# Medical-Image-Analysis-Laboratory/fetal_t2mapping

Measured on AMD Instinct MI355X. Metric: Mvoxel/s T2 fit, 256³×8TE 3-param LM, 1/2/4/8 GPU; % HBM roofline, higher is better.
Workload: dtype f64

## Files before the change

fetal_t2mapping_amd/csrc/t2fit_kernels.hip:

```cpp
#include <hip/hip_runtime.h>

#include <algorithm>
#include <atomic>
#include <cstdlib>
#include <string>

#include "t2fit_config.h"
#include "t2fit_diag.h"
#include "t2fit_dispatch.h"
#include "t2fit_error.h"
#include "t2fit_launch.h"
#include "t2fit_support.h"

using namespace t2fit;

namespace {

constexpr int kLdsStride = kBlock + 1;
#ifndef T2_SAMPLE_LOAD
#define T2_SAMPLE_LOAD(p) (*(p))
#endif
#ifndef T2_WAVE_HINT
#define T2_WAVE_HINT 2
#endif
constexpr int kWaveHint = T2_WAVE_HINT;

struct Tuning {
  bool use_persistent = true;
  int persistent_blocks = 2048;
  int refill_min = 0;
  bool nte_special = true;
  int take = 0;
  int64_t small_volume = 1 << 20;
  int wave_wg = 1;
  int waves_per_cu = 0;
};
std::atomic<bool> g_reserve_set{false};
std::atomic<int> g_reserve_cus{0};

const Tuning& tuning() {
  static const Tuning tuned = [] {
    Tuning t;
    if (const char* e = std::getenv("T2FIT_ONE_SHOT")) t.use_persistent = std::atoi(e) == 0;
    if (const char* e = std::getenv("T2FIT_PERSISTENT_BLOCKS")) t.persistent_blocks = std::max(1, std::atoi(e));
    if (const char* e = std::getenv("T2FIT_REFILL_MIN")) t.refill_min = std::min(64, std::max(1, std::atoi(e)));
    if (const char* e = std::getenv("T2FIT_RESERVE_CUS"); e && !g_reserve_set.load()) g_reserve_cus.store(std::max(0, std::atoi(e)));
    if (const char* e = std::getenv("T2FIT_NTE_SPECIAL")) t.nte_special = std::atoi(e) != 0;
    if (const char* e = std::getenv("T2FIT_TAKE")) t.take = std::max(0, std::min(64, std::atoi(e)));
    if (const char* e = std::getenv("T2FIT_SMALL_VOLUME")) t.small_volume = std::max<int64_t>(0, std::atoll(e));
    if (const char* e = std::getenv("T2FIT_WAVE_WG")) t.wave_wg = std::max(0, std::atoi(e));
    if (const char* e = std::getenv("T2FIT_WAVES_PER_CU")) t.waves_per_cu = std::max(0, std::atoi(e));
    return t;
  }();
  return tuned;
}

thread_local bool g_timing = false;
constexpr int kEvRing = 16;
thread_local hipEvent_t g_ev0[kEvRing] = {}, g_ev1[kEvRing] = {}, g_ev2[kEvRing] = {};
thread_local long g_ev_count = 0;
thread_local int g_ev_slot = 0;

double event_ms(int launches_ago, const hipEvent_t* from, const hipEvent_t* to) {
  if (launches_ago < 0 || launches_ago >= kEvRing || launches_ago >= g_ev_count) return -1.0;
  const int slot = (int)((g_ev_count - 1 - launches_ago) % kEvRing);
  if (hipEventSynchronize(to[slot]) != hipSuccess) return -1.0;
  float ms = 0.0f;
  if (hipEventElapsedTime(&ms, from[slot], to[slot]) != hipSuccess) return -1.0;
  return (double)ms;
}

struct DevMaps {
  float *t2, *k, *sigma, *res, *r2, *fun, *se;
  int32_t* nit;
  uint8_t* status;
  double* xd;
  double* fund;
  double* trace = nullptr;
  int32_t* trace_len = nullptr;
  int trace_cap = 0;
};

__device__ __forceinline__ void stage_echoes(float* lds, const float* __restrict__ echoes, int layout,
                                             int n_te, int64_t n_vox, int64_t base, bool load_own) {
  const int lane = threadIdx.x;
  if (layout == T2FIT_LAYOUT_TE_MAJOR) {
    if (load_own) {
      const float* src = echoes + base + lane;
      for (int i = 0; i < n_te; ++i) lds[i * kLdsStride + lane] = src[(int64_t)i * n_vox];
    }
  } else {
    const int64_t rows = n_vox - base < kBlock ? n_vox - base : kBlock;
    const int total = (int)rows * n_te;
    const float* src = echoes + base * n_te;
    for (int j = lane; j < total; j += kBlock) {
      const int v = j / n_te;
      const int i = j - v * n_te;
      lds[i * kLdsStride + v] = src[j];
    }
    __syncthreads();
  }
}

template <bool kExtras = true, bool kEpilogueFollows = false>
__device__ __forceinline__ void store_masked(const DevMaps& m, int64_t v) {
  m.t2[v] = 0.0f; m.k[v] = 0.0f; m.sigma[v] = 0.0f;
  if constexpr (!kEpilogueFollows) m.res[v] = 0.0f;
  if constexpr (!kExtras) return;
  if constexpr (!kEpilogueFollows) {
    if (m.r2) m.r2[v] = 0.0f;
    if (m.se) m.se[v] = 0.0f;
  }
  if (m.fun) m.fun[v] = 0.0f;
  if (m.nit) m.nit[v] = 0;
  if (m.status) m.status[v] = T2FIT_ST_MASKED;
  if (m.xd) { m.xd[3 * v] = 0.0; m.xd[3 * v + 1] = 0.0; m.xd[3 * v + 2] = 0.0; }
  if (m.fund) m.fund[v] = 0.0;
}

__device__ __forceinline__ void store_result(const DevMaps& m, int64_t v, const LaneOutputs& o, const LaneResult& r) {
  m.t2[v] = o.t2; m.k[v] = o.k; m.sigma[v] = o.sigma; m.res[v] = o.res;
  if (m.r2) m.r2[v] = o.r2;
  if (m.se) m.se[v] = o.se;
  if (m.fun) m.fun[v] = o.fun;
  if (m.nit) m.nit[v] = o.nit;
  if (m.status) m.status[v] = o.status;
  if (m.xd) { m.xd[3 * v] = r.x[0]; m.xd[3 * v + 1] = r.x[1]; m.xd[3 * v + 2] = r.x[2]; }
  if (m.fund) m.fund[v] = r.fun;
}

template <bool kExtras = true>
__device__ __forceinline__ void store_fit(const DevMaps& m, int64_t v, const LaneResult& r) {
  m.k[v] = (float)r.x[0]; m.t2[v] = (float)r.x[1]; m.sigma[v] = (float)r.x[2];
  if constexpr (!kExtras) return;
  if (m.fun) m.fun[v] = (float)r.fun;
  if (m.nit) m.nit[v] = r.nit;
  if (m.status) m.status[v] = r.status;
  if (m.xd) { m.xd[3 * v] = r.x[0]; m.xd[3 * v + 1] = r.x[1]; m.xd[3 * v + 2] = r.x[2]; }
  if (m.fund) m.fund[v] = r.fun;
}

template <int SOLVER, int PREC, int MODEL>
__global__ __launch_bounds__(kBlock) void fit_volume_kernel(const LaneParams P, const float* __restrict__ echoes,
                                                            int layout, const uint8_t* __restrict__ mask,
                                                            int64_t n_vox, DevMaps m) {
  extern __shared__ float lds[];
  const int lane = threadIdx.x;
  const int64_t base = (int64_t)blockIdx.x * kBlock;
  const int64_t v = base + lane;
  const bool in_range = v < n_vox;
  const bool active = in_range && (mask == nullptr || mask[v] != 0);
  stage_echoes(lds, echoes, layout, P.n_te, n_vox, base, active);
  if (!in_range) return;
  if (!active) {
    store_masked(m, v);
    return;
  }
  bool finite;
  float y0_raw;
  const ObjCtx c = prepare_samples(P, lds + lane, kLdsStride, finite, y0_raw);
  LaneResult r;
  fit_lane_t<SOLVER, PREC, MODEL>(P, c, finite, y0_raw, r);
  LaneOutputs o;
  lane_epilogue(c, r, o, m.r2 != nullptr, m.se != nullptr);
  store_result(m, v, o, r);
}

constexpr int kLoglinVec = 4;
constexpr int kLoglinTile = kBlock * kLoglinVec;

template <bool kExtras>
__global__ __launch_bounds__(kBlock) void loglin_volume_kernel(const LaneParams P, const float* __restrict__ echoes,
                                                               const uint8_t* __restrict__ mask, int64_t n_vox,
                                                               DevMaps m) {
  extern __shared__ float lds[];
  const int lane = threadIdx.x;
  const int64_t v0 = (int64_t)blockIdx.x * kLoglinTile + (int64_t)lane * kLoglinVec;
  if (v0 >= n_vox) return;
  const int n_te = P.n_te;
  bool act[kLoglinVec] = {true, true, true, true};
  if (mask) {
    const uchar4 mk = *reinterpret_cast<const uchar4*>(mask + v0);
    act[0] = mk.x != 0; act[1] = mk.y != 0; act[2] = mk.z != 0; act[3] = mk.w != 0;
  }
  const bool any = act[0] || act[1] || act[2] || act[3];
  bool fin[kLoglinVec] = {true, true, true, true};
  float ymax[kLoglinVec] = {0.0f, 0.0f, 0.0f, 0.0f}, y0[kLoglinVec] = {0.0f, 0.0f, 0.0f, 0.0f};
  if (any) {
    const float* src = echoes + v0;
    for (int i0 = 0; i0 < n_te; i0 += 8) {
      float4 tmp[8];
#pragma unroll
      for (int j = 0; j < 8; ++j)
        if (i0 + j < n_te) tmp[j] = *reinterpret_cast<const float4*>(src + (int64_t)(i0 + j) * n_vox);
#pragma unroll
      for (int j = 0; j < 8; ++j)
        if (i0 + j < n_te) {
          float* dst = lds + (i0 + j) * kLoglinTile + lane;
          const float sv[kLoglinVec] = {tmp[j].x, tmp[j].y, tmp[j].z, tmp[j].w};
#pragma unroll
          for (int q = 0; q < kLoglinVec; ++q) {
            dst[q * kBlock] = sv[q];
            fin[q] = fin[q] && t2_finite(sv[q]);
            if (i0 + j == 0) { y0[q] = sv[q]; ymax[q] = sv[q]; }
            ymax[q] = sv[q] > ymax[q] ? sv[q] : ymax[q];
          }
        }
    }
  }
  float o_t2[kLoglinVec], o_k[kLoglinVec], o_res[kLoglinVec];
  const bool want_fun = kExtras && (m.fun != nullptr || m.fund != nullptr);
#pragma unroll
  for (int q = 0; q < kLoglinVec; ++q) {
    o_t2[q] = 0.0f; o_k[q] = 0.0f; o_res[q] = 0.0f;
    const int64_t v = v0 + q;
    if (!act[q]) {
      if constexpr (kExtras) {
        if (m.r2) m.r2[v] = 0.0f;
        if (m.se) m.se[v] = 0.0f;
        if (m.fun) m.fun[v] = 0.0f;
        if (m.nit) m.nit[v] = 0;
        if (m.status) m.status[v] = T2FIT_ST_MASKED;
        if (m.xd) { m.xd[3 * v] = 0.0; m.xd[3 * v + 1] = 0.0; m.xd[3 * v + 2] = 0.0; }
        if (m.fund) m.fund[v] = 0.0;
      }
      continue;
    }
    float* col = lds + q * kBlock + lane;
    bool finite = fin[q];
    if (P.norm) {
      for (int i = 0; i < n_te; ++i) {
        const float sv = col[i * kLoglinTile] / ymax[q];
        col[i * kLoglinTile] = sv;
        finite = finite && t2_finite(sv);
      }
    }
    ObjCtx c;
    c.P = &P;
    c.y = EchoView{col, kLoglinTile};
    double lb[3], ub[3];
    const bool feasible = lane_bounds(P, y0[q], lb, ub);
    LaneResult r;
    r.nit = 0; r.nfev = 0; r.fun = NAN;
    if (!feasible) {
      r.x[0] = NAN; r.x[1] = NAN; r.x[2] = 0.0;
      r.status = T2FIT_ST_INFEASIBLE;
    } else if (!finite) {
      r.x[0] = t2_clip(P.x0[0], lb[0], ub[0]); r.x[1] = t2_clip(P.x0[1], lb[1], ub[1]); r.x[2] = 0.0;
      r.status = T2FIT_ST_NONFINITE;
    } else {
      loglin_solve(c, lb, ub, want_fun, r);
    }
    LaneOutputs o;
    lane_epilogue(c, r, o, kExtras && m.r2 != nullptr, kExtras && m.se != nullptr);
    o_t2[q] = o.t2; o_k[q] = o.k; o_res[q] = o.res;
    if constexpr (kExtras) {
      if (m.r2) m.r2[v] = o.r2;
      if (m.se) m.se[v] = o.se;
      if (m.fun) m.fun[v] = o.fun;
      if (m.nit) m.nit[v] = o.nit;
      if (m.status) m.status[v] = o.status;
      if (m.xd) { m.xd[3 * v] = r.x[0]; m.xd[3 * v + 1] = r.x[1]; m.xd[3 * v + 2] = r.x[2]; }
      if (m.fund) m.fund[v] = r.fun;
    }
  }
  *reinterpret_cast<float4*>(m.t2 + v0) = make_float4(o_t2[0], o_t2[1], o_t2[2], o_t2[3]);
  *reinterpret_cast<float4*>(m.k + v0) = make_float4(o_k[0], o_k[1], o_k[2], o_k[3]);
  *reinterpret_cast<float4*>(m.sigma + v0) = make_float4(0.0f, 0.0f, 0.0f, 0.0f);
  *reinterpret_cast<float4*>(m.res + v0) = make_float4(o_res[0], o_res[1], o_res[2], o_res[3]);
}

constexpr int kChunkLarge = 256;
constexpr int kChunkSmall = 64;
constexpr int kQueueCap = 64 + kChunkLarge;

template <int MODEL, int NTE = 0, int HOME = PAIRS_LDS> struct LbfgsbLane {
  using Solver = Lbfgsb<MODEL, NTE, HOME>;
  using WaveWg = LbfgsbLane<MODEL, NTE, MODEL == T2FIT_MODEL_GAUSSIAN ? PAIRS_LDS
                                         : MODEL == T2FIT_MODEL_RICIAN ? PAIRS_GLOBAL : PAIRS_REG>;
  static constexpr bool kGlobalPart = Solver::kPairGlobal;
  static constexpr int NP = Solver::N;
  static constexpr int kNte = NTE;
  static constexpr int kHistDoubles = Solver::M * Solver::PAIR_L;
  static constexpr int kWavesPerSimd = 1;
  static constexpr bool kWaveWgOk = true;
#ifndef T2_WAVE_HINT_2PAR
#define T2_WAVE_HINT_2PAR 3
#endif
  static constexpr int kWaveWgHint = MODEL == T2FIT_MODEL_GAUSSIAN ? T2_WAVE_HINT_2PAR : kWaveHint;
  static constexpr int kRefillMin = MODEL == T2FIT_MODEL_RICIAN ? 4 : 8;
  static constexpr bool kSplit = true;
  __device__ static void init(Solver& s, const ObjCtx&, const double* x0, const double* lb, const double* ub,
                              double* hist, int hstride, double* ghist) { s.init(x0, lb, ub, hist, hstride, ghist, 64); }
  __device__ static void result(const Solver& s, const ObjCtx&, LaneResult& r) { s.result(r); }
  template <int J> __device__ static void take_sample(Solver& s, float y) {
    if constexpr (NTE > 0 && J < NTE) s.ys[J] = y;
  }
};
template <typename T, int NPAR, int NTE = 0> struct LmLaneAdaptor {
  using Solver = LmLane<T, NPAR, NTE>;
  using WaveWg = LmLaneAdaptor<T, NPAR, NTE>;
  static constexpr bool kGlobalPart = false;
  static constexpr int NP = NPAR;
  static constexpr int kNte = NTE;
  static constexpr int kHistDoubles = 0;
  static constexpr bool kWaveWgOk = false;
  static constexpr int kWaveWgHint = 1;
  static constexpr int kWavesPerSimd = sizeof(T) == 4 ? 4 : 1;
  static constexpr int kRefillMin = 24;
  static constexpr bool kSplit = false;
  __device__ static void init(Solver& s, const ObjCtx& c, const double* x0, const double* lb, const double* ub,
                              double*, int, double*) { s.init(c, x0, lb, ub); }
  __device__ static void result(const Solver& s, const ObjCtx& c, LaneResult& r) { s.result(c, r); }
  template <int J> __device__ static void take_sample(Solver&, float) {}
};

template <class A, int kChunk, bool kTrace, bool kExtras, int kWg = kBlock, bool kRegs = false>
__device__ __forceinline__ void persistent_fit(const LaneParams& P, const float* __restrict__ echoes, int layout,
                                               const uint8_t* __restrict__ mask, int64_t n_vox, const DevMaps& m,
                                               unsigned long long* next_chunk, int refill_min, int take, double* ghist_all) {
  extern __shared__ float lds[];
  constexpr int NP = A::NP;
  constexpr bool kWaveWg = kRegs;
  static_assert(kRegs ? (kChunk == 64 && A::kNte > 0 && A::kNte <= 8) : kWg == kBlock,
                "workgroup of 256 lanes, or waves taking 64-voxel chunks with the samples in registers");
  constexpr int kStride = kWaveWg ? 64 : kLdsStride;
  const int lane = threadIdx.x & 63, wave = threadIdx.x >> 6;
  float* col = lds + threadIdx.x;
  double* hist = reinterpret_cast<double*>(lds + (kWaveWg ? 0 : ((P.n_te * kStride + 1) & ~1))) + threadIdx.x;
  uint32_t* queue = reinterpret_cast<uint32_t*>(hist - threadIdx.x + A::kHistDoubles * kWg) + wave * kQueueCap;
  double* ghist = nullptr;
  if constexpr (A::kGlobalPart)
    ghist = ghist_all + ((size_t)blockIdx.x * (kWg / 64) + wave) * (A::Solver::M * 64) + lane;
  uint32_t qv = 0;
  const unsigned long long lt_mask = lane == 0 ? 0ull : (~0ull >> (64 - lane));
  const EchoView y{col, kStride};
  int q_head = 0, q_count = 0;
  bool chunks_left = true;
  bool busy = false, done = false;
  int64_t v = 0;
  typename A::Solver s;
  ObjCtx c;
  c.P = &P;
  c.y = y;
  double box_x0[3], box_lb[3], box_ub[3];
#pragma unroll
  for (int j = 0; j < 3; ++j) { box_x0[j] = P.x0[j]; box_lb[j] = P.lb[j]; box_ub[j] = P.ub[j]; }
  T2_STAMPS_BEGIN(queue - wave * kQueueCap + (kBlock / 64) * kQueueCap, wave, lane, c)
  T2_RECORD_PLACEMENT(next_chunk, blockIdx.x * (kWg / 64) + wave, lane)
  bool parked = false;
  int pend = 0;
  const int kTake = take;
  int64_t base_a = 0;
  int sub_a = 0;
  uint32_t idx_b = 0;
  uint8_t mask_a = 0;
  auto load_mask = [&](int64_t base) -> uint8_t {
    const int64_t vv = base + lane;
    return vv < n_vox ? (mask ? mask[vv] : (uint8_t)1) : (uint8_t)0;
  };
  if constexpr (kWaveWg) {
    uint32_t c0 = 0;
    if (lane == 0) c0 = (uint32_t)atomicAdd(next_chunk, 1ull);
    base_a = (int64_t)__shfl(c0, 0, 64) * (64 * kTake);
    mask_a = load_mask(base_a);
    if (lane == 0) idx_b = (uint32_t)atomicAdd(next_chunk, 1ull);
  }
  for (;;) {
    unsigned long long need = __ballot(!busy);
    if (__popcll(need) >= refill_min || need == ~0ull) {
      do {
      T2_BLK_T0(t_rf)
      if (done) {
        LaneResult r;
        A::result(s, c, r);
        store_fit<kExtras>(m, v, r);
        done = false;
      }
      bool fresh = false;
      if constexpr (kWaveWg) {
        unsigned long long want = need;
        for (;;) {
          if (q_count == 0) {
            if (!chunks_left) break;
            const int64_t base = base_a;
            if (base >= n_vox) { chunks_left = false; break; }
            const int64_t vv = base + lane;
            const bool act = mask_a != 0;
            if (++sub_a < kTake) {
              base_a += 64;
              mask_a = load_mask(base_a);
            } else {
              sub_a = 0;
              base_a = (int64_t)__shfl(idx_b, 0, 64) * (64 * kTake);
              mask_a = load_mask(base_a);
              if (lane == 0) idx_b = (uint32_t)atomicAdd(next_chunk, 1ull);
            }
            const unsigned long long b = __ballot(act);
            q_count = __popcll(b);
            q_head = 0;
            const int dst = act ? __popcll(b & lt_mask) : q_count + __popcll(~b & lt_mask);
            qv = (uint32_t)__builtin_amdgcn_ds_permute(dst << 2, (int)(uint32_t)vv);
            if (vv < n_vox && !act) store_masked<kExtras, true>(m, vv);
            if (q_count == 0) continue;
          }
          const int rank = __popcll(want & lt_mask);
          const uint32_t got = (uint32_t)__builtin_amdgcn_ds_bpermute(((q_head + rank) & 63) << 2, (int)qv);
          if (!busy && rank < q_count) {
            v = (int64_t)got;
            busy = true;
            fresh = true;
          }
          const int n_want = __popcll(want);
          const int taken = n_want < q_count ? n_want : q_count;
          q_head += taken;
          q_count -= taken;
          want = __ballot(!busy);
          if (want == 0ull) break;
        }
      } else {
      const int n_need = __popcll(need);
      while (q_count < n_need && chunks_left) {
        unsigned long long cidx = 0;
        if (lane == 0) cidx = atomicAdd(next_chunk, 1ull);
        cidx = __shfl(cidx, 0, 64);
        const int64_t base = (int64_t)cidx * kChunk;
        if (base >= n_vox) { chunks_left = false; break; }
        if (q_head != 0) {
          uint32_t tmp = 0;
          if (lane < q_count) tmp = queue[q_head + lane];
          if (lane < q_count) queue[lane] = tmp;
          q_head = 0;
        }
        bool act[kChunk / 64];
#pragma unroll
        for (int q = 0; q < kChunk / 64; ++q) {
          const int64_t vv = base + q * 64 + lane;
          act[q] = vv < n_vox && (mask == nullptr || mask[vv] != 0);
        }
#pragma unroll
        for (int q = 0; q < kChunk / 64; ++q) {
          const unsigned long long b = __ballot(act[q]);
          if (act[q]) queue[q_count + __popcll(b & lt_mask)] = (uint32_t)(base + q * 64 + lane);
          q_count += __popcll(b);
        }
#pragma unroll
        for (int q = 0; q < kChunk / 64; ++q) {
          const int64_t vv = base + q * 64 + lane;
          if (vv < n_vox && !act[q]) store_masked<kExtras, true>(m, vv);
        }
      }
      if (!busy) {
        const int rank = __popcll(need & lt_mask);
        if (rank < q_count) {
          v = (int64_t)queue[q_head + rank];
          busy = true;
          fresh = true;
        }
      }
      const int taken = n_need < q_count ? n_need : q_count;
      q_head += taken;
      q_count -= taken;
      }
      if (fresh) {
        bool finite = true;
        float ymax = 0.0f, y0 = 0.0f;
        const int n_te = A::kNte > 0 ? A::kNte : P.n_te;
        float first8[8] = {};
        for (int i0 = 0; i0 < n_te; i0 += 8) {
          float tmp[8];
#pragma unroll
          for (int j = 0; j < 8; ++j)
            if (i0 + j < n_te)
              tmp[j] = T2_SAMPLE_LOAD(layout == T2FIT_LAYOUT_TE_MAJOR ? &echoes[(int64_t)(i0 + j) * n_vox + v]
                                                                      : &echoes[v * n_te + (i0 + j)]);
#pragma unroll
          for (int j = 0; j < 8; ++j)
            if (i0 + j < n_te) {
              const float sv = tmp[j];
              if constexpr (!kWaveWg) col[(i0 + j) * kStride] = sv;
              if (i0 == 0) first8[j] = sv;
              finite = finite && t2_finite(sv);
              if (i0 + j == 0) { y0 = sv; ymax = sv; }
              ymax = sv > ymax ? sv : ymax;
            }
        }
        if (P.norm) {
          if constexpr (A::kNte > 0) {
#pragma unroll
            for (int j = 0; j < 8; ++j)
              if (j < n_te) {
                const float sv = first8[j] / ymax;
                first8[j] = sv;
                if constexpr (!kWaveWg) col[j * kStride] = sv;
                finite = finite && t2_finite(sv);
              }
          } else {
            for (int i = 0; i < n_te; ++i) {
              const float sv = col[i * kStride] / ymax;
              col[i * kStride] = sv;
              finite = finite && t2_finite(sv);
            }
          }
        }
        if constexpr (A::kNte > 0)
          static_for<0, 8>([&](auto JC) { A::template take_sample<decltype(JC)::value>(s, first8[decltype(JC)::value]); });
        double lb[3], ub[3];
#pragma unroll
        for (int j = 0; j < 3; ++j) { lb[j] = box_lb[j]; ub[j] = box_ub[j]; }
        if (P.no_prior) {
          lb[0] = (double)y0; ub[0] = P.np_k_ub;
          lb[1] = P.np_t2_lb; ub[1] = P.np_t2_ub;
        }
        bool feasible = true;
#pragma unroll
        for (int j = 0; j < NP; ++j) feasible = feasible && !(lb[j] > ub[j]);
        if (!feasible || !finite) {
          LaneResult r;
          r.nit = 0; r.nfev = 0; r.fun = NAN;
          for (int j = 0; j < 3; ++j)
            r.x[j] = !feasible ? (j < NP ? NAN : 0.0) : (j < NP ? t2_clip(box_x0[j], lb[j], ub[j]) : 0.0);
          r.status = !feasible ? T2FIT_ST_INFEASIBLE : T2FIT_ST_NONFINITE;
          store_fit<kExtras>(m, v, r);
          busy = false;
        } else {
          if constexpr (kTrace) {
            c.trace = m.trace + (size_t)v * 4 * m.trace_cap;
            c.trace_cap = m.trace_cap;
            c.trace_n = m.trace_len + v;
            *c.trace_n = 0;
          }
          A::init(s, c, box_x0, lb, ub, hist, kWg, ghist);
          if constexpr (A::kSplit) { T2_STAMPS_ATTACH(s) }
        }
      }
      T2_BLK_END(c, 8, t_rf)
      need = __ballot(!busy);
      } while (need == ~0ull && (chunks_left || q_count != 0));
    }
    if (__ballot(busy) == 0ull) break;
    if constexpr (A::kSplit) {
      if (busy) {
        if (!parked) {
          T2_BLK_T0(t_ev)
          s.eval(c);
          T2_BLK_END(c, 7, t_ev)
          pend = s.digest(c);
        }
        if (pend == A::Solver::GO_BEGIN || pend == A::Solver::GO_FAIL) {
          T2_BLK_T0(t_bg)
          pend = s.begin_pass(c, pend);
          T2_BLK_END(c, 9, t_bg)
        }
        parked = pend == A::Solver::GO_BEGIN || pend == A::Solver::GO_FAIL;
        if (pend == A::Solver::GO_DONE) { busy = false; done = true; }
      }
    } else {
      if (busy) s.eval(c);
      if (busy && s.advance(c)) {
        busy = false;
        done = true;
      }
    }
  }
  if (done) {
    LaneResult r;
    A::result(s, c, r);
    store_fit<kExtras>(m, v, r);
  }
  T2_STAMPS_END(next_chunk, lane)
}

template <class A, int kChunk, bool kTrace = false, int kWavesPerSimd = 1, bool kExtras = true, int kWg = kBlock,
          bool kRegs = false>
__global__ __launch_bounds__(kWg, kWavesPerSimd) void fit_persistent_kernel(const LaneParams P,
                                                                    const float* __restrict__ echoes, int layout,
                                                                    const uint8_t* __restrict__ mask, int64_t n_vox,
                                                                    DevMaps m, unsigned long long* next_chunk, int refill_min,
                                                                    int take, double* ghist) {
  persistent_fit<A, kChunk, kTrace, kExtras, kWg, kRegs>(P, echoes, layout, mask, n_vox, m, next_chunk, refill_min, take, ghist);
}

__global__ __launch_bounds__(kBlock) void residuals_kernel(const LaneParams P, const float* __restrict__ echoes,
                                                           int layout, const uint8_t* __restrict__ mask,
                                                           int64_t n_vox, const float* __restrict__ t2,
                                                           const float* __restrict__ k,
                                                           const float* __restrict__ sigma, float* res, float* r2,
                                                           float* se) {
  extern __shared__ float lds[];
  const int lane = threadIdx.x;
  const int64_t base = (int64_t)blockIdx.x * kBlock;
  const int64_t v = base + lane;
  const bool in_range = v < n_vox;
  const bool active = in_range && (mask == nullptr || mask[v] != 0);
  stage_echoes(lds, echoes, layout, P.n_te, n_vox, base, active);
  if (!in_range) return;
  float out = 0.0f, out2 = 0.0f, out3 = 0.0f;
  if (active) {
    bool finite;
    float y0_raw;
    const ObjCtx c = prepare_samples(P, lds + lane, kLdsStride, finite, y0_raw);
    const float kv = k[v], tv = t2[v], sv = sigma ? sigma[v] : 0.0f;
    out = residual_mean(c, kv, tv, sv);
    if (r2) out2 = r_squared(c, (double)kv, (double)tv, (double)sv);
    if (se) out3 = t2_std_error(c, (double)kv, (double)tv, (double)sv);
  }
  res[v] = out;
  if (r2) r2[v] = out2;
  if (se) se[v] = out3;
}

using FitKernel = void (*)(const LaneParams, const float*, int, const uint8_t*, int64_t, DevMaps);

FitKernel pick_kernel(const t2fit_config& c) {
  if (c.solver == T2FIT_SOLVER_LM) {
// ... 259 lines not shown
```

fetal_t2mapping_amd/csrc/t2fit_lane.h:

```cpp
#pragma once

#include <math.h>
#include <stdint.h>

#include <type_traits>

#include "../../include/t2fit.h"
#include "t2fit_diag.h"

#if defined(__HIPCC__)
#define T2_HD __host__ __device__ __forceinline__
#define T2_DEVICE_COMPILE 1
#define T2_UNROLL _Pragma("unroll")
#else
#define T2_HD inline
#define T2_UNROLL
#endif

namespace t2fit {

struct LaneParams {
  int32_t model, solver, precision, n_te;
  int32_t no_prior, norm, maxls, maxiter, maxfun, numpy_legacy;
  double te[T2FIT_MAX_TE];
// ... 82 lines not shown
  double r = fma(-0x1.62e42fefa39efp-1, n, x);
  r = fma(-0x1.abc9e3b39803fp-56, n, r);
  double p = fma(0x1.ade156a5dcb37p-26, r, 0x1.28af3fca7ab0cp-22);
  p = fma(r, p, 0x1.71dee623fde64p-19);
  p = fma(r, p, 0x1.a01997c89e6b0p-16);
  p = fma(r, p, 0x1.a01a014761f6ep-13);
  p = fma(r, p, 0x1.6c16c1852b7b0p-10);
  p = fma(r, p, 0x1.1111111122322p-7);
  p = fma(r, p, 0x1.55555555502a1p-5);
  p = fma(r, p, 0x1.5555555555511p-3);
  p = fma(r, p, 0x1.000000000000bp-1);
  p = fma(r, p, 1.0);
  p = fma(r, p, 1.0);
  return __builtin_ldexp(p, (int)n);
}
T2_HD double t2_sqrt_core(double x) {
  const double y = fmin(__builtin_amdgcn_rsq(x), 1e300);
  double g = x * y, h = y * 0.5;
  const double r = fma(-h, g, 0.5);
  g = fma(g, r, g);
  double d = fma(-g, g, x);
  h = fma(h, r, h);
  g = fma(d, h, g);
  d = fma(-g, g, x);
  g = fma(d, h, g);
  return g;
}
#else
T2_HD double t2_exp_core(double x) { return exp(x); }
T2_HD double t2_sqrt_core(double x) { return sqrt(x); }
#endif

T2_HD double t2_sqrt_from_seed_seq(double x, double y, double& h_out) {
  double g = x * y, h = y * 0.5;
  const double r = fma(-h, g, 0.5);
  g = fma(g, r, g);
  double d = fma(-g, g, x);
  h = fma(h, r, h);
  g = fma(d, h, g);
  d = fma(-g, g, x);
  g = fma(d, h, g);
  h_out = h;
  return g;
}
T2_HD double t2_rsqrt_half_near_seq(double a, double h) {
  const double g = a * (h + h);
  return fma(h, fma(-h, g, 0.5), h);
}
T2_HD double t2_sqrt_near_seq(double a, double h) {
  double g = a * (h + h);
  const double r = fma(-h, g, 0.5);
  g = fma(g, r, g);
  const double hi = fma(h, r, h);
  const double d = fma(-g, g, a);
  return fma(d, hi, g);
}
T2_HD double t2_sqrt_from_h_seq(double a, double h) {
  const double g0 = a * (h + h);
  return fma(fma(-g0, g0, a), h, g0);
}
#if defined(__HIP_DEVICE_COMPILE__)
T2_HD double t2_sqrt_core_h(double x, double& h_out) { return t2_sqrt_from_seed_seq(x, __builtin_amdgcn_rsq(x), h_out); }
T2_HD double t2_sqrt_near(double a, double h) { return t2_sqrt_near_seq(a, h); }
T2_HD double t2_rsqrt_half_near(double a, double h) { return t2_rsqrt_half_near_seq(a, h); }
T2_HD double t2_sqrt_from_h(double a, double h) { return t2_sqrt_from_h_seq(a, h); }
#else
T2_HD double t2_sqrt_core_h(double x, double& h_out) { h_out = 0.5 / sqrt(x); return sqrt(x); }
T2_HD double t2_sqrt_near(double a, double) { return sqrt(a); }
T2_HD double t2_rsqrt_half_near(double a, double) { return 0.5 / sqrt(a); }
T2_HD double t2_sqrt_from_h(double a, double) { return sqrt(a); }
#endif

template <typename T> T2_HD T t2_min(T a, T b) { return a < b ? a : b; }
template <typename T> T2_HD T t2_max(T a, T b) { return a > b ? a : b; }
template <typename T> T2_HD T t2_clip(T x, T lo, T hi) {
  T r = x;
  if (lo > r) r = lo;
  if (hi < r) r = hi;
  return r;
}
template <typename T> T2_HD T t2_abs(T a) { return a < T(0) ? -a : a; }
T2_HD bool t2_finite(double x) { return (x - x) == 0.0; }
T2_HD bool t2_finite(float x) { return (x - x) == 0.0f; }

template <typename T> struct TeOf;
template <> struct TeOf<double> {
  T2_HD static double at(const LaneParams& P, int i) { return P.te[i]; }
};
template <> struct TeOf<float> {
  T2_HD static float at(const LaneParams& P, int i) { return P.te_f[i]; }
};

template <int J, int JN, class F> T2_HD void static_for(F&& f) {
  if constexpr (J < JN) {
    f(std::integral_constant<int, J>{});
    static_for<J + 1, JN>(f);
  }
}

#if defined(__HIPCC__)
#define T2_TABLE __device__ __constant__
#else
#define T2_TABLE static const
#endif
T2_TABLE double t2_i0e_A[30] = {
    -4.41534164647933937950E-18, 3.33079451882223809783E-17,  -2.43127984654795469359E-16,
    1.71539128555513303061E-15,  -1.16853328779934516808E-14, 7.67618549860493561688E-14,
    -4.85644678311192946090E-13, 2.95505266312963983461E-12,  -1.72682629144155570723E-11,
    9.67580903537323691224E-11,  -5.18979560163526290666E-10, 2.65982372468238665035E-9,
    -1.30002500998624804212E-8,  6.04699502254191894932E-8,   -2.67079385394061173391E-7,
    1.11738753912010371815E-6,   -4.41673835845875056359E-6,  1.64484480707288970893E-5,
    -5.75419501008210370398E-5,  1.88502885095841655729E-4,   -5.76375574538582365885E-4,
    1.63947561694133579842E-3,   -4.32430999505057594430E-3,  1.05464603945949983183E-2,
    -2.37374148058994688156E-2,  4.93052842396707084878E-2,   -9.49010970480476444210E-2,
    1.71620901522208775349E-1,   -3.04682672343198398683E-1,  6.76795274409476084995E-1};
T2_TABLE double t2_i0e_B[25] = {
    -7.23318048787475395456E-18, -4.83050448594418207126E-18, 4.46562142029675999901E-17,
    3.46122286769746109310E-17,  -2.82762398051658348494E-16, -3.42548561967721913462E-16,
    1.77256013305652638360E-15,  3.81168066935262242075E-15,  -9.55484669882830764870E-15,
    -4.15056934728722208663E-14, 1.54008621752140982691E-14,  3.85277838274214270114E-13,
    7.18012445138366623367E-13,  -1.79417853150680611778E-12, -1.32158118404477131188E-11,
    -3.14991652796324136454E-11, 1.18891471078464383424E-11,  4.94060238822496958910E-10,
    3.39623202570838634515E-9,   2.26666899049817806459E-8,   2.04891858946906374183E-7,
    2.89137052083475648297E-6,   6.88975834691682398426E-5,   3.36911647825569408990E-3,
    8.04490411014108831608E-1};

#if defined(T2_I0E_FMA)
#define T2_CLENSHAW(z, b1, b2, c) (fma(z, b1, -(b2)) + (c))
#else
#define T2_CLENSHAW(z, b1, b2, c) ((z) * (b1) - (b2) + (c))
#endif
#if defined(__HIP_DEVICE_COMPILE__)
#define T2_NOUNROLL _Pragma("nounroll")
#define T2_WAVE_ANY(p) (__ballot(p) != 0ull)
#else
#define T2_NOUNROLL
#define T2_WAVE_ANY(p) (p)
#endif

T2_HD double t2_chbevl(double x, const double* c, int n) {
  double b0 = c[0], b1 = 0.0, b2 = 0.0;
  for (int i = 1; i < n; ++i) {
    b2 = b1;
    b1 = b0;
    b0 = x * b1 - b2 + c[i];
  }
  return 0.5 * (b0 - b2);
}

T2_HD double t2_i0e(double x) {
  if (x < 0) x = -x;
  if (x <= 8.0) return t2_chbevl(x * 0.5 - 2.0, t2_i0e_A, 30);
  return t2_fdiv(t2_chbevl(t2_fdiv(32.0, x) - 2.0, t2_i0e_B, 25), t2_sqrt_core(x));
}

T2_HD void t2_chbevl4(const double* z, const double* tab, int chunks, double* out) {
  double b0[4], b1[4], b2[4];
  T2_UNROLL
  for (int j = 0; j < 4; ++j) { b0[j] = 0.0; b1[j] = 0.0; b2[j] = 0.0; }
  double cn[5];
  T2_UNROLL
  for (int q = 0; q < 5; ++q) cn[q] = tab[q];
  T2_NOUNROLL
  for (int it = 0; it < chunks; ++it) {
    double cc[5];
    T2_UNROLL
// ... 295 lines not shown
```

fetal_t2mapping_amd/csrc/t2fit_lbfgsb.h:

```cpp
#pragma once

#include <type_traits>

#include "t2fit_lane.h"

namespace t2fit {

template <int MODEL> struct ObjTerm;
T2_HD double rician_log_term(float log_y, double log_s2, bool legacy) {
  return legacy ? (double)(log_y - (float)log_s2) : (double)log_y - log_s2;
}
template <> struct ObjTerm<T2FIT_MODEL_GAUSSIAN> {
  double k, t2;
  T2_HD void set(const ObjCtx&, const double* x) { k = x[0]; t2 = x[1]; }
  T2_HD double at(const ObjCtx& c, int i) const {
    const double r = (double)c.sample(i) - k * t2_exp_core(t2_fdiv(-c.P->te[i], t2));
    return r * r;
  }
  T2_HD double finish(const ObjCtx& c, double s) const { return s / c.P->n_te; }
};
template <> struct ObjTerm<T2FIT_MODEL_GAUSSIAN_RICIAN> {
  double k2, t2, s2;
  T2_HD void set(const ObjCtx&, const double* x) { k2 = x[0] * x[0]; t2 = x[1]; s2 = x[2] * x[2]; }
  T2_HD double at(const ObjCtx& c, int i) const {
// ... 692 lines not shown
    T2_UNROLL
    for (int i = 0; i < N; ++i) { fr[i] = iwhere[i] <= 0; nfree += fr[i]; du[i] = 0.0; }
    T2_UNROLL
    for (int i = 0; i < N; ++i) {
      double bz = 0.0;
      T2_UNROLL
      for (int j = 0; j < N; ++j) bz = fma(B[i][j], z[j] - x[j], bz);
      r[i] = fr[i] ? -(g[i] + bz) : 0.0;
    }
    double A[3][3] = {{1, 0, 0}, {0, 1, 0}, {0, 0, 1}};
    T2_UNROLL
    for (int i = 0; i < N; ++i)
      T2_UNROLL
      for (int j = 0; j < N; ++j)
        if (fr[i] && fr[j]) A[i][j] = B[i][j];
    double rr[3] = {r[0], r[1], N == 3 ? r[N - 1] : 0.0};
    if (N == 2) rr[2] = 0.0;
    const double d0 = A[0][0], r0 = t2_fast_rcp(d0);
    const double l10 = A[1][0] * r0, l20 = A[2][0] * r0;
    const double d1 = fma(-l10, A[1][0], A[1][1]), r1 = t2_fast_rcp(d1);
    const double a21 = fma(-l20, A[1][0], A[2][1]);
    const double l21 = a21 * r1;
    const double d2 = fma(-l21, a21, fma(-l20, A[2][0], A[2][2])), r2 = t2_fast_rcp(d2);
    const bool pos_def = (d0 > 0.0) & (d1 > 0.0) & (d2 > 0.0);
    const double y0 = rr[0], y1 = fma(-l10, y0, rr[1]), y2 = fma(-l21, y1, fma(-l20, y0, rr[2]));
    const double u2 = y2 * r2, u1 = fma(-l21, u2, y1 * r1);
    const double u0 = fma(-l20, u2, fma(-l10, u1, y0 * r0));
    du[0] = u0; du[1] = u1;
    if (N == 3) du[N - 1] = u2;
    double xp[N];
    bool projected = false;
    T2_UNROLL
    for (int i = 0; i < N; ++i) {
      xp[i] = z[i];
      const double xk = lb_min(ub[i], lb_max(lb[i], z[i] + du[i]));
      z[i] = fr[i] ? xk : z[i];
      projected = projected | (fr[i] & ((xk == lb[i]) | (xk == ub[i])));
    }
    double ddp = 0.0;
    T2_UNROLL
    for (int i = 0; i < N; ++i) ddp = fma(z[i] - x[i], g[i], ddp);
    if (projected && ddp > 0.0) {
      T2_UNROLL
      for (int i = 0; i < N; ++i) z[i] = xp[i];
      double alpha = 1.0, temp1 = 1.0;
      bool hit[N];
      T2_UNROLL
      for (int i = 0; i < N; ++i) hit[i] = false;
      T2_UNROLL
      for (int i = 0; i < N; ++i) {
        if (fr[i]) {
          const double dk = du[i];
          if (dk < 0.0) {
            const double temp2 = lb[i] - z[i];
            if (temp2 >= 0.0) temp1 = 0.0;
            else if (dk * alpha < temp2) temp1 = t2_fdiv(temp2, dk);
          } else if (dk > 0.0) {
            const double temp2 = ub[i] - z[i];
            if (temp2 <= 0.0) temp1 = 0.0;
            else if (dk * alpha > temp2) temp1 = t2_fdiv(temp2, dk);
          }
          if (temp1 < alpha) {
            alpha = temp1;
            T2_UNROLL
            for (int j = 0; j < N; ++j) hit[j] = j == i;
          }
        }
      }
      if (alpha < 1.0) {
        T2_UNROLL
        for (int i = 0; i < N; ++i)
          if (hit[i]) {
            if (du[i] > 0.0) { z[i] = ub[i]; du[i] = 0.0; }
            else if (du[i] < 0.0) { z[i] = lb[i]; du[i] = 0.0; }
          }
      }
      T2_UNROLL
      for (int i = 0; i < N; ++i)
        if (fr[i]) z[i] = fma(alpha, du[i], z[i]);
    }
    return pos_def;
  }

  T2_HD void init(const double* x0_, const double* lb_, const double* ub_, double* hist_, int hstride_,
                  double* ghist_ = nullptr, int gstride_ = 0) {
    hist = hist_;
    hstride = hstride_;
    ghist = ghist_;
    gstride = gstride_;
    head = 0;
    T2_UNROLL
    for (int i = 0; i < N; ++i) {
      lb[i] = lb_[i];
      ub[i] = ub_[i];
      x[i] = t2_clip(x0_[i], lb[i], ub[i]);
      iwhere[i] = (ub[i] - lb[i] <= 0.0) ? 3 : 0;
    }
    col = 0; nit = 0; nfev = 0; ifun = 0;
    theta = 1.0;
    status = T2FIT_ST_NOT_CONV;
    first = true;
    wn_stale = false;
    T2_UNROLL
    for (int i = 0; i < N; ++i) { z[i] = 0.0; d[i] = 0.0; t[i] = 0.0; r[i] = 0.0; g[i] = 0.0; }
    f = 0.0; fold = 0.0; gd = 0.0; gdold = 0.0; stp = 1.0; stpmx = 1.0; sbgnrm = 0.0;
    ls.task = LS_START; ls.stage = 1; ls.brackt = false;
    ls.ginit = ls.gtest = ls.gx = ls.gy = ls.finit = ls.fx = ls.fy = 0.0;
    ls.stx = ls.sty = ls.stmin = ls.stmax = ls.width = ls.width1 = 0.0;
  }

  enum { GO_BEGIN, GO_TRIAL, GO_FAIL, GO_DONE };

  T2_HD int digest(const ObjCtx& c) {
    const LaneParams& P = *c.P;
    const double epsmch = 2.220446049250313e-16;
    T2_BLK_T0(t_dig)
    const bool was_first = first;
    first = false;
    double gdn = 0.0;
    T2_UNROLL
    for (int i = 0; i < N; ++i) gdn += g[i] * d[i];
    LsState lsn = ls;
    const int task = dcsrch_tests(f, gdn, stp, 0.9, 0.1, 0.0, stpmx, lsn);
    const bool cont = !was_first & (task == LS_FG);
    const bool newit = !was_first & (task != LS_FG);
    double stpn = stp;
    dcsrch_update(f, gdn, stpn, 0.1, 0.0, stpmx, lsn);
    const double sb = projgr(x, g);
    const double tol = P.lbfgsb_tol;
    const int nit1 = nit + 1;
    const bool out_of_budget = (nit1 >= P.maxiter) | (nfev > P.maxfun);
    const bool converged = (sb <= P.gtol) | (!was_first & ((fold - f) <= tol * t2_max3(lb_abs(fold), lb_abs(f), 1.0)));
    double rn[N], dn[N], rr = 0.0;
    T2_UNROLL
    for (int i = 0; i < N; ++i) { rn[i] = g[i] - r[i]; rr += rn[i] * rn[i]; }
    const double dr = (gdn - gdold) * stp, ddum = -gdold * stp;
    T2_UNROLL
    for (int i = 0; i < N; ++i) dn[i] = d[i] * stp;
    const double theta_n = t2_fdiv(rr, dr);
    const double rsy = t2_fast_rsqrt(dr);
    const bool iterate_on = newit & !out_of_budget & !converged;
    const bool store_pair = iterate_on & !(dr <= epsmch * ddum);
    if (!was_first) gd = gdn;
    if (cont) { ls = lsn; stp = stpn; ++ifun; }
    if (!cont && !was_first) ls.task = lsn.task;
    if (was_first || newit) sbgnrm = sb;
    if (newit) {
      nit = nit1;
      if (c.trace && *c.trace_n < c.trace_cap) {
        double* tr = c.trace + 4 * (*c.trace_n)++;
        tr[0] = x[0]; tr[1] = x[1]; tr[2] = N == 3 ? x[N - 1] : 0.0; tr[3] = f;
      }
    }
    if (iterate_on) {
      T2_UNROLL
      for (int i = 0; i < N; ++i) { r[i] = rn[i]; d[i] = dn[i]; }
    }
    if (store_pair) {
      if (col == M) {
        head = (head + 1) % M;
        col = M - 1;
      }
      const int q = slot_of(col);
      store_s(q, dn);
      T2_UNROLL
      for (int i = 0; i < N; ++i) hy(q, i) = rn[i] * rsy;
      ++col;
      theta = theta_n;
    }
    if ((was_first || newit) && converged && !(newit && out_of_budget)) status = T2FIT_ST_CONVERGED;
    const int next_ls = ifun - 1 >= P.maxls ? GO_FAIL : GO_TRIAL;
    const int next_it = (converged | (!was_first & out_of_budget)) ? GO_DONE : GO_BEGIN;
    const int next = cont ? next_ls : next_it;
    T2_BLK_END(c, 0, t_dig)
    set_trial(next == GO_TRIAL);
    return next;
  }

  T2_HD void set_trial(bool on = true) {
    T2_UNROLL
    for (int i = 0; i < N; ++i) {
      const double xt = stp * d[i] + t[i];
      x[i] = on ? (stp == 1.0 ? z[i] : xt) : x[i];
    }
  }
// ... 98 lines not shown
```

Baseline: 1629.

## Streamline wave-workgroup refill: 32-bit offsets, early sample loads, skip scratch zeroing

In the wave-per-workgroup L-BFGS-B path, the refill step now issues the echo sample loads before storing the previous voxel's result, so memory latency overlaps the stores. It uses 32-bit byte offsets for map stores and TE-major sample loads when the volume has fewer than 2^30 voxels, and replaces per-sample finiteness checks with a bitwise max-magnitude test. Solver scratch state is zeroed once per lane rather than on every voxel init, and the refill threshold for non-Rician models drops from 8 to 6. The change depends on the solver never reading stale scratch values between voxels, and adds code paths for the two offset and layout cases.

```diff
diff --git a/fetal_t2mapping_amd/csrc/t2fit_kernels.hip b/fetal_t2mapping_amd/csrc/t2fit_kernels.hip
--- a/fetal_t2mapping_amd/csrc/t2fit_kernels.hip
+++ b/fetal_t2mapping_amd/csrc/t2fit_kernels.hip
@@ -102,9 +102,14 @@
   }
 }
 
-template <bool kExtras = true, bool kEpilogueFollows = false>
+template <bool kOff32> __device__ __forceinline__ float& map_at(float* map, int64_t v) {
+  if constexpr (kOff32) return *reinterpret_cast<float*>(reinterpret_cast<char*>(map) + ((uint32_t)v << 2));
+  else return map[v];
+}
+
+template <bool kExtras = true, bool kEpilogueFollows = false, bool kOff32 = false>
 __device__ __forceinline__ void store_masked(const DevMaps& m, int64_t v) {
-  m.t2[v] = 0.0f; m.k[v] = 0.0f; m.sigma[v] = 0.0f;
+  map_at<kOff32>(m.t2, v) = 0.0f; map_at<kOff32>(m.k, v) = 0.0f; map_at<kOff32>(m.sigma, v) = 0.0f;
   if constexpr (!kEpilogueFollows) m.res[v] = 0.0f;
   if constexpr (!kExtras) return;
   if constexpr (!kEpilogueFollows) {
@@ -129,9 +134,9 @@
   if (m.fund) m.fund[v] = r.fun;
 }
 
-template <bool kExtras = true>
+template <bool kExtras = true, bool kOff32 = false>
 __device__ __forceinline__ void store_fit(const DevMaps& m, int64_t v, const LaneResult& r) {
-  m.k[v] = (float)r.x[0]; m.t2[v] = (float)r.x[1]; m.sigma[v] = (float)r.x[2];
+  map_at<kOff32>(m.k, v) = (float)r.x[0]; map_at<kOff32>(m.t2, v) = (float)r.x[1]; map_at<kOff32>(m.sigma, v) = (float)r.x[2];
   if constexpr (!kExtras) return;
   if (m.fun) m.fun[v] = (float)r.fun;
   if (m.nit) m.nit[v] = r.nit;
@@ -288,10 +293,14 @@
 #define T2_WAVE_HINT_2PAR 3
 #endif
   static constexpr int kWaveWgHint = MODEL == T2FIT_MODEL_GAUSSIAN ? T2_WAVE_HINT_2PAR : kWaveHint;
-  static constexpr int kRefillMin = MODEL == T2FIT_MODEL_RICIAN ? 4 : 8;
+  static constexpr int kRefillMin = MODEL == T2FIT_MODEL_RICIAN ? 4 : 6;
   static constexpr bool kSplit = true;
+  template <bool kZeroScratch = true>
   __device__ static void init(Solver& s, const ObjCtx&, const double* x0, const double* lb, const double* ub,
-                              double* hist, int hstride, double* ghist) { s.init(x0, lb, ub, hist, hstride, ghist, 64); }
+                              double* hist, int hstride, double* ghist) {
+    s.template init<kZeroScratch>(x0, lb, ub, hist, hstride, ghist, 64);
+  }
+  __device__ static void clear(Solver& s) { s.clear_scratch(); }
   __device__ static void result(const Solver& s, const ObjCtx&, LaneResult& r) { s.result(r); }
   template <int J> __device__ static void take_sample(Solver& s, float y) {
     if constexpr (NTE > 0 && J < NTE) s.ys[J] = y;
@@ -309,8 +318,10 @@
   static constexpr int kWavesPerSimd = sizeof(T) == 4 ? 4 : 1;
   static constexpr int kRefillMin = 24;
   static constexpr bool kSplit = false;
+  template <bool = true>
   __device__ static void init(Solver& s, const ObjCtx& c, const double* x0, const double* lb, const double* ub,
                               double*, int, double*) { s.init(c, x0, lb, ub); }
+  __device__ static void clear(Solver&) {}
   __device__ static void result(const Solver& s, const ObjCtx& c, LaneResult& r) { s.result(c, r); }
   template <int J> __device__ static void take_sample(Solver&, float) {}
 };
@@ -340,6 +351,7 @@
   bool busy = false, done = false;
   int64_t v = 0;
   typename A::Solver s;
+  if constexpr (kWaveWg) A::clear(s);
   ObjCtx c;
   c.P = &P;
   c.y = y;
@@ -359,6 +371,7 @@
     const int64_t vv = base + lane;
     return vv < n_vox ? (mask ? mask[vv] : (uint8_t)1) : (uint8_t)0;
   };
+  const bool off32 = kWaveWg && n_vox < ((int64_t)1 << 30);
   if constexpr (kWaveWg) {
     uint32_t c0 = 0;
     if (lane == 0) c0 = (uint32_t)atomicAdd(next_chunk, 1ull);
@@ -371,12 +384,15 @@
     if (__popcll(need) >= refill_min || need == ~0ull) {
       do {
       T2_BLK_T0(t_rf)
-      if (done) {
-        LaneResult r;
-        A::result(s, c, r);
-        store_fit<kExtras>(m, v, r);
-        done = false;
-      }
+      if constexpr (!kWaveWg) {
+        if (done) {
+          LaneResult r;
+          A::result(s, c, r);
+          store_fit<kExtras>(m, v, r);
+          done = false;
+        }
+      }
+      const int64_t v_done = v;
       bool fresh = false;
       if constexpr (kWaveWg) {
         unsigned long long want = need;
@@ -401,7 +417,10 @@
             q_head = 0;
             const int dst = act ? __popcll(b & lt_mask) : q_count + __popcll(~b & lt_mask);
             qv = (uint32_t)__builtin_amdgcn_ds_permute(dst << 2, (int)(uint32_t)vv);
-            if (vv < n_vox && !act) store_masked<kExtras, true>(m, vv);
+            if (vv < n_vox && !act) {
+              if (off32) store_masked<kExtras, true, true>(m, vv);
+              else store_masked<kExtras, true>(m, vv);
+            }
             if (q_count == 0) continue;
           }
           const int rank = __popcll(want & lt_mask);
@@ -462,11 +481,55 @@
       q_head += taken;
       q_count -= taken;
       }
-      if (fresh) {
-        bool finite = true;
-        float ymax = 0.0f, y0 = 0.0f;
+      bool finite = true;
+      float y0 = 0.0f;
+      float first8[8] = {};
+      if constexpr (kWaveWg) {
+        constexpr int n_te = A::kNte;
+        if (fresh) {
+          if (off32 && layout == T2FIT_LAYOUT_TE_MAJOR) {
+            int64_t plane_bytes = n_vox * (int64_t)sizeof(float);
+            asm volatile("" : "+s"(plane_bytes));
+            const char* plane = reinterpret_cast<const char*>(echoes);
+            const uint32_t off = (uint32_t)v << 2;
+#pragma unroll
+            for (int j = 0; j < 8; ++j)
+              if (j < n_te) {
+                first8[j] = T2_SAMPLE_LOAD(reinterpret_cast<const float*>(plane + off));
+                plane += plane_bytes;
+              }
+          } else {
+#pragma unroll
+            for (int j = 0; j < 8; ++j)
+              if (j < n_te)
+                first8[j] = T2_SAMPLE_LOAD(layout == T2FIT_LAYOUT_TE_MAJOR ? &echoes[(int64_t)j * n_vox + v] : &echoes[v * n_te + j]);
+#pragma unroll
+            for (int j = 0; j < 8; ++j)
+              if (j < n_te) asm volatile("" : : "v"(first8[j]));
+          }
+        }
+        if (done) {
+          LaneResult r;
+          A::result(s, c, r);
+          if (off32) store_fit<kExtras, true>(m, v_done, r);
+          else store_fit<kExtras>(m, v_done, r);
+          done = false;
+        }
+        if (fresh) {
+          finite = t2_all_finite<n_te>(first8);
+          y0 = first8[0];
+          if (P.norm) {
+            float ymax = first8[0];
+#pragma unroll
+            for (int j = 1; j < n_te; ++j) ymax = first8[j] > ymax ? first8[j] : ymax;
+#pragma unroll
+            for (int j = 0; j < n_te; ++j) first8[j] = first8[j] / ymax;
+            finite = finite && t2_all_finite<n_te>(first8);
+          }
+        }
+      } else if (fresh) {
+        float ymax = 0.0f;
         const int n_te = A::kNte > 0 ? A::kNte : P.n_te;
-        float first8[8] = {};
         for (int i0 = 0; i0 < n_te; i0 += 8) {
           float tmp[8];
 #pragma unroll
@@ -478,7 +541,7 @@
           for (int j = 0; j < 8; ++j)
             if (i0 + j < n_te) {
               const float sv = tmp[j];
-              if constexpr (!kWaveWg) col[(i0 + j) * kStride] = sv;
+              col[(i0 + j) * kStride] = sv;
               if (i0 == 0) first8[j] = sv;
               finite = finite && t2_finite(sv);
               if (i0 + j == 0) { y0 = sv; ymax = sv; }
@@ -492,7 +555,7 @@
               if (j < n_te) {
                 const float sv = first8[j] / ymax;
                 first8[j] = sv;
-                if constexpr (!kWaveWg) col[j * kStride] = sv;
+                col[j * kStride] = sv;
                 finite = finite && t2_finite(sv);
               }
           } else {
@@ -503,6 +566,8 @@
             }
           }
         }
+      }
+      if (fresh) {
         if constexpr (A::kNte > 0)
           static_for<0, 8>([&](auto JC) { A::template take_sample<decltype(JC)::value>(s, first8[decltype(JC)::value]); });
         double lb[3], ub[3];
@@ -521,7 +586,8 @@
           for (int j = 0; j < 3; ++j)
             r.x[j] = !feasible ? (j < NP ? NAN : 0.0) : (j < NP ? t2_clip(box_x0[j], lb[j], ub[j]) : 0.0);
           r.status = !feasible ? T2FIT_ST_INFEASIBLE : T2FIT_ST_NONFINITE;
-          store_fit<kExtras>(m, v, r);
+          if (off32) store_fit<kExtras, true>(m, v, r);
+          else store_fit<kExtras>(m, v, r);
           busy = false;
         } else {
           if constexpr (kTrace) {
@@ -530,7 +596,7 @@
             c.trace_n = m.trace_len + v;
             *c.trace_n = 0;
           }
-          A::init(s, c, box_x0, lb, ub, hist, kWg, ghist);
+          A::template init<!kWaveWg>(s, c, box_x0, lb, ub, hist, kWg, ghist);
           if constexpr (A::kSplit) { T2_STAMPS_ATTACH(s) }
         }
       }
diff --git a/fetal_t2mapping_amd/csrc/t2fit_lane.h b/fetal_t2mapping_amd/csrc/t2fit_lane.h
--- a/fetal_t2mapping_amd/csrc/t2fit_lane.h
+++ b/fetal_t2mapping_amd/csrc/t2fit_lane.h
@@ -188,6 +188,15 @@
 template <typename T> T2_HD T t2_abs(T a) { return a < T(0) ? -a : a; }
 T2_HD bool t2_finite(double x) { return (x - x) == 0.0; }
 T2_HD bool t2_finite(float x) { return (x - x) == 0.0f; }
+template <int N> T2_HD bool t2_all_finite(const float* p) {
+  uint32_t top = 0;
+  T2_UNROLL
+  for (int i = 0; i < N; ++i) {
+    const uint32_t mag = __builtin_bit_cast(uint32_t, p[i]) & 0x7fffffffu;
+    top = mag > top ? mag : top;
+  }
+  return top < 0x7f800000u;
+}
 
 template <typename T> struct TeOf;
 template <> struct TeOf<double> {
diff --git a/fetal_t2mapping_amd/csrc/t2fit_lbfgsb.h b/fetal_t2mapping_amd/csrc/t2fit_lbfgsb.h
--- a/fetal_t2mapping_amd/csrc/t2fit_lbfgsb.h
+++ b/fetal_t2mapping_amd/csrc/t2fit_lbfgsb.h
@@ -798,6 +798,7 @@
     return pos_def;
   }
 
+  template <bool kZeroScratch = true>
   T2_HD void init(const double* x0_, const double* lb_, const double* ub_, double* hist_, int hstride_,
                   double* ghist_ = nullptr, int gstride_ = 0) {
     hist = hist_;
@@ -817,6 +818,10 @@
     status = T2FIT_ST_NOT_CONV;
     first = true;
     wn_stale = false;
+    if constexpr (kZeroScratch) clear_scratch();
+  }
+
+  T2_HD void clear_scratch() {
     T2_UNROLL
     for (int i = 0; i < N; ++i) { z[i] = 0.0; d[i] = 0.0; t[i] = 0.0; r[i] = 0.0; g[i] = 0.0; }
     f = 0.0; fold = 0.0; gd = 0.0; gdold = 0.0; stp = 1.0; stpmx = 1.0; sbgnrm = 0.0;
```

Result: slower. 1475 (-9.5%).
